# databio/IGD

Measured on AMD Instinct MI355X. Metric: query-intervals/sec (igd search -q, hits-only) on roadmap-scale synthetic .igd, higher is better.
Workload: dtype int32; 1 GPU; BASELINE config 2: roadmap-scale synthetic IGD, 1900 files x 26316 intervals (53143736 tile records, 188505 tiles of 16384 bp, hg38 contigs) replicated per GPU + 1000000 position-sorted queries per step (seed 7), hits-only, queries and DB resident in HBM; queries_per_gpu=1000000, parallelism=query-sharded x1, grouping=sorted, query_layout=contig numbers + starts + ends (12 B/query; igd_hip_search_dev), collective=none

## Files before the change

### igd_amd/csrc/engine/host_search.hpp

```cpp

static int ensure_workspace(igd_hip_db *db, int64_t nq, int pairBytes)
{
    int rc;
    if (nq > db->wsQueries) {
        HIPCHK(hipDeviceSynchronize());
        if (db->d_fix) (void)hipFree(db->d_fix);
        if (db->d_qw) (void)hipFree(db->d_qw);
        if (db->d_later) (void)hipFree(db->d_later);
        if (db->d_laterHdr) (void)hipFree(db->d_laterHdr);
        db->d_fix = nullptr; db->d_qw = nullptr; db->d_later = nullptr; db->d_laterHdr = nullptr;
        db->wsQueries = 0;
        if ((rc = dalloc(&db->d_fix, (size_t)nq * 2, nullptr)) != IGD_HIP_OK) return rc;
        if ((rc = dalloc(&db->d_qw, (size_t)nq + 64, nullptr)) != IGD_HIP_OK) return rc;
        if ((rc = dalloc(&db->d_later, (size_t)nq + 4096 + 64, nullptr)) != IGD_HIP_OK) return rc;
        if ((rc = dalloc(&db->d_laterHdr, 2 * ((size_t)nq / 256 + 2), nullptr)) != IGD_HIP_OK) return rc;
        db->wsQueries = nq;
    }
    if (pairBytes == 0 || (nq <= db->wsBucket && pairBytes <= db->pairBytes)) return IGD_HIP_OK;
    HIPCHK(hipDeviceSynchronize());
    const int64_t cap = nq > db->wsBucket ? nq : db->wsBucket;
    const int pb = pairBytes > db->pairBytes ? pairBytes : db->pairBytes;
    {
        void *ws[] = { db->d_pairs, db->d_long, db->d_spTable, db->d_spT, db->d_spSub };
        for (void *q : ws) if (q) (void)hipFree(q);
// ... 168 lines not shown
                                       int64_t *d_hits, int64_t *d_total, void *stream)
{
    if (!d_run_start || (flags & IGD_HIP_FLAG_BUCKET)) {
        snprintf(g_err, sizeof g_err, "igd_hip_search_runs_dev: bad argument");
        return IGD_HIP_ERR_ARG;
    }
    return search_dev_impl(db, nullptr, d_run_start, d_qs, d_qe, nq, v, rule, flags | IGD_HIP_FLAG_SORTED, d_hits, d_total, stream);
}

static int search_dev_impl(igd_hip_db *db, const int32_t *d_ichr, const int32_t *d_runs, const int32_t *d_qs,
                           const int32_t *d_qe, int64_t nq, int32_t v, int rule, int flags,
                           int64_t *d_hits, int64_t *d_total, void *stream)
{
    if (!db || !d_hits || nq < 0 || nq > IGD_MAX_BATCH || (rule != IGD_HIP_RULE_NEST && rule != IGD_HIP_RULE_FLAT) ||
        ((flags & IGD_HIP_FLAG_SORTED) && (flags & IGD_HIP_FLAG_BUCKET))) {
        snprintf(g_err, sizeof g_err, "igd_hip_search_dev: bad argument");
        return IGD_HIP_ERR_ARG;
    }
    if (db->nFiles == 0) return IGD_HIP_OK;
    if (db->inner) {
        db->inner->vnest = rule == IGD_HIP_RULE_NEST ? 1 : 0;
        return search_dev_impl(db->inner, d_ichr, d_runs, d_qs, d_qe, nq, v, IGD_HIP_RULE_FLAT, flags, d_hits, d_total,
                               stream ? stream : (void *)db->stream);
    }
    HIPCHK(hipSetDevice(db->device));
    hipStream_t st = stream ? (hipStream_t)stream : db->stream;
    if (nq == 0 || db->nT == 0) {
        if (flags & IGD_HIP_FLAG_ZERO_FIRST) {
            HIPCHK(hipMemsetAsync(d_hits, 0, (size_t)db->nFiles * 8, st));
            if (d_total) HIPCHK(hipMemsetAsync(d_total, 0, 8, st));
        }
        return IGD_HIP_OK;
    }
    int rc = ensure_workspace(db, nq, (flags & IGD_HIP_FLAG_SORTED) ? 0 : 8);
    if (rc != IGD_HIP_OK) return rc;
    const bool useV = (v != IGD_HIP_NO_VALUE_FILTER && db->gType == 1);
    const int mode = (flags & IGD_HIP_FLAG_SORTED) ? 1 : (flags & IGD_HIP_FLAG_BUCKET) ? 2 : 0;
    const int krule = rule | ((db->v.vshift >= 0 && db->vnest) ? 0x100 : 0);
    const bool packed = db->packed && !(flags & IGD_HIP_FLAG_EXACT) && (!useV || db->packedV);
    if (db->epoch >= 0x3fffffff || db->covStale) {
        HIPCHK(hipMemsetAsync(db->d_spill, 0, ((size_t)db->nT + 2) * 4, st));
        HIPCHK(hipMemsetAsync(db->d_cov, 0, 4 * IGD_COV_LEN(db->nT) * 4, st));
        HIPCHK(hipMemsetAsync(db->d_ctl + CTL_COV, 0, 4 * 4, st));
        if (db->d_spSub && db->spShift >= 0)
            HIPCHK(hipMemsetAsync(db->d_spSub + (((size_t)db->spCoarse * SPF_S) << db->spShift) + db->spCoarse, 0, (size_t)db->spCoarse * 4, st));
        if (!db->covStale) db->epoch = 0;
        db->covStale = false;
    }
    db->epoch++;
    struct StaleGuard { igd_hip_db *d; bool done; ~StaleGuard() { if (!done) d->covStale = true; } } guard{db, false};
    int slot = -1;
    if (db->evOn && db->evUsed < db->evMax && (db->evSeen++ % (db->evEvery > 0 ? db->evEvery : 1)) == 0) slot = db->evUsed++;
    const bool pipeEv = slot >= 0 && slot < IGD_PIPE_EVENTS;
    if (pipeEv) HIPCHK(hipEventRecord(db->ev[4 * slot + 0], st));
    u64 *zh = (flags & IGD_HIP_FLAG_ZERO_FIRST) ? (u64 *)d_hits : nullptr;
    u64 *zt = (flags & IGD_HIP_FLAG_ZERO_FIRST) ? (u64 *)d_total : nullptr;
    const bool direct = mode == 1 && packed && db->ldsHits && db->nWin == 1 && db->v.tileD != nullptr && db->v.vshift < 0 && db->v.shift >= 0 && db->nCtg <= QB_CTG &&
                        (db->forceDirect > 0 || (db->forceDirect < 0 && (flags & IGD_HIP_FLAG_SHORT) && nq >= 28ll * db->nT));
    db->lastDirect = direct ? 1 : 0;
    if (mode != 2) {
        bool vec = ((((uintptr_t)d_ichr) | ((uintptr_t)d_qs) | ((uintptr_t)d_qe)) & 15) == 0;
        const bool fast = packed && db->v.shift >= 0 && db->nCtg <= QB_CTG;
        if (nq < 65536) vec = false;
        bool runsK = d_runs != nullptr && vec && fast;
        if (d_runs && !runsK) {
            if (nq > db->runCap) {
                HIPCHK(hipStreamSynchronize(st));
                if (db->d_runIchr) (void)hipFree(db->d_runIchr);
                db->d_runIchr = nullptr; db->runCap = 0;
                if ((rc = dalloc(&db->d_runIchr, (size_t)nq, nullptr)) != IGD_HIP_OK) return rc;
                db->runCap = nq;
            }
            k_expand_runs<<<(int)((nq + 255) / 256), 256, 0, st>>>(d_runs, db->nCtg, db->d_runIchr, (int)nq);
            d_ichr = db->d_runIchr;
            vec = vec && (((uintptr_t)d_ichr) & 15) == 0;
        }
        const int fillBlocks = (int)((db->nT >> 10) < 256 ? (db->nT >> 10) + 1 : 256);
        const bool wide = vec && nq >= ((int64_t)1 << 22);
#define QB_GRID(PER_) ((int)((nq + (PER_) - 1) / (PER_)) > fillBlocks ? (int)((nq + (PER_) - 1) / (PER_)) : fillBlocks)
#define QB_LAUNCH(VEC_, FAST_, WGT_)                                                                                                  \
    if (direct && FAST_ && runsK && VEC_ == 4)                                         \
        k_query_bounds<4, true, WGT_, true, true><<<QB_GRID(WGT_ * 4), WGT_, 0, st>>>(db->v, d_runs, d_qs, d_qe, (int)nq, krule,      \
        1, db->d_firstQ, db->d_lpos, db->d_fix, db->d_ctl, db->epoch, zh, zt, db->d_qw, db->d_later, db->d_spill,                      \
        (int2 *)db->d_laterHdr, 1);                                                                                                  \
    else if (direct && FAST_)                                                                                                        \
        k_query_bounds<VEC_, true, WGT_, false, true><<<QB_GRID(WGT_ * VEC_), WGT_, 0, st>>>(db->v, d_ichr, d_qs, d_qe, (int)nq, krule, \
        1, db->d_firstQ, db->d_lpos, db->d_fix, db->d_ctl, db->epoch, zh, zt, db->d_qw, db->d_later, db->d_spill,                      \
        (int2 *)db->d_laterHdr, 1);                                                                                                  \
    else if (runsK && VEC_ == 4 && FAST_)                                                                                             \
        k_query_bounds<4, true, WGT_, true><<<QB_GRID(WGT_ * 4), WGT_, 0, st>>>(db->v, d_runs, d_qs, d_qe, (int)nq, krule,            \
        packed ? 1 : 0, db->d_firstQ, db->d_lpos, db->d_fix, db->d_ctl, db->epoch, zh, zt, db->d_qw, db->d_later, db->d_spill,         \
        (int2 *)db->d_laterHdr, mode == 1 ? 1 : 0);                                                                                  \
    else                                                                                                                             \
    k_query_bounds<VEC_, FAST_, WGT_><<<QB_GRID(WGT_ * VEC_), WGT_, 0, st>>>(db->v, d_ichr, d_qs, d_qe, (int)nq, krule,               \
        packed ? 1 : 0, db->d_firstQ, db->d_lpos, db->d_fix, db->d_ctl, db->epoch, zh, zt, db->d_qw, db->d_later, db->d_spill,         \
        (int2 *)db->d_laterHdr, mode == 1 ? 1 : 0)
        if (wide && !direct) { if (fast) QB_LAUNCH(4, true, 1024); else QB_LAUNCH(4, false, 1024); }
        else if (vec) { if (fast) QB_LAUNCH(4, true, 256); else QB_LAUNCH(4, false, 256); }
        else { if (fast) QB_LAUNCH(1, true, 256); else QB_LAUNCH(1, false, 256); }
#undef QB_LAUNCH
#undef QB_GRID
        db->lbShift = wide ? 12 : vec ? 10 : 8;
    }
    if (mode != 1) {
        if (db->spShift >= 0)
            rc = launch_split(db, d_ichr, d_qs, d_qe, (int)nq, krule, mode == 2 ? 0 : db->epoch, packed ? 1 : 0, st,
                              mode == 2 ? zh : nullptr, mode == 2 ? zt : nullptr);
        else
            rc = launch_bucket(db, d_ichr, d_qs, d_qe, (int)nq, krule, mode == 2 ? 0 : db->epoch, packed ? 1 : 0, st,
                                      mode == 2 ? zh : nullptr, mode == 2 ? zt : nullptr);
        if (rc != IGD_HIP_OK) return rc;
    }
    const bool extEv = slot >= 0 && mode == 1 && packed && db->ldsHits && db->nWin == 1;
    if (slot >= 0 && !extEv) HIPCHK(hipEventRecord(db->ev[4 * slot + 1], st));
    ScanArgs a;
    a.firstQ = db->d_firstQ; a.pairN = db->d_pairN; a.pairPos = db->d_pairPos; a.pairs = (const int2 *)db->d_pairs;
    a.walkList = nullptr; a.ctl = db->d_ctl; a.q_ichr = d_ichr; a.q_qs = d_qs; a.q_qe = d_qe; a.q_w = db->d_qw;
    a.total = (u64 *)d_total; a.hitsOut = (u64 *)d_hits;
    a.nq = (int)nq; a.v = v; a.rule = rule; a.epoch = db->epoch; a.mode = mode;
    a.packedWalk = packed ? (useV ? 2 : 1) : 0;
    const int valves = direct ? 8 : (mode != 1 && packed && db->spShift >= 0 ? 1 : 0) | (mode != 2 && packed ? 2 : 0) |
                       (db->bigImage || db->nRec + IGD_CHUNK >= (1ll << 30) ? 4 : 0);
    const size_t tailWave = direct ? (size_t)IGD_D_WLDS : (size_t)IGD_WLDS_BYTES;
    size_t tailLds = (valves & (2 | 8)) ? (size_t)(db->ldsHits ? IGD_TAIL_WG / IGD_WAVE : 4) * tailWave : 0;
    int tailHistOff = -1;
    if ((size_t)db->nFiles * 8 <= (size_t)48 * 1024) { tailHistOff = (int)tailLds; tailLds += (size_t)db->nFiles * 8; }
    if (db->ldsHits) {
        a.out = db->d_slab;
        const SortK K = make_sortk(db, a);
        for (int win = 0; win < db->nWin; win++) {
            const bool last = win == db->nWin - 1;
            const int fileLo = win * db->winN, fileN = db->nWin == 1 ? db->nFiles : (db->nFiles - fileLo < db->winN ? db->nFiles - fileLo : db->winN);
            if (extEv) { db->evStart = db->ev[4 * slot + 1]; db->evStop = db->ev[4 * slot + 2]; }
            if (direct) {
                DirK D;
                D.db = db->v;
                D.a.firstQ = db->d_firstQ; D.a.tileD = db->v.tileD; D.a.q_qs = d_qs; D.a.q_qe = d_qe; D.a.ctl = db->d_ctl; D.a.fix = db->d_fix;
                D.a.heavyS = db->d_heavy + IGD_HEAVY_MAX; D.a.farList = db->d_far; D.a.nq = (int)nq; D.a.v = v; D.a.epoch = db->epoch;
                D.a.rule = rule; D.a.promised = 1; D.a.sbCap = db->sbCap; D.a.wldsBytes = IGD_D_WLDS + 2 * db->sbCap;
                D.a.out = db->d_slab; D.a.hitsOut = (u64 *)d_hits; D.a.totalOut = (u64 *)d_total;
                if (useV) launch_sorted(db, igd_scan_direct<true>, db->grid, IGD_WG_DIR, (size_t)db->ldsDirect, st, D);
                else launch_sorted(db, igd_scan_direct<false>, db->grid, IGD_WG_DIR, (size_t)db->ldsDirect, st, D);
            } else
            launch_scan_any<true>(db, a, useV, packed, st, db->nWin > 1 ? win : -1);
            if (extEv && db->evStart) {
                db->evStart = db->evStop = nullptr;
                HIPCHK(hipEventRecord(db->ev[4 * slot + 1], st)); HIPCHK(hipEventRecord(db->ev[4 * slot + 2], st));
            }
            if (slot >= 0 && last && !extEv) HIPCHK(hipEventRecord(db->ev[4 * slot + 2], st));
            ScanArgs w = a;
            w.out = (u64 *)d_hits;
            SortK Kt = K;
            Kt.a.sbCap = 0; Kt.a.wldsBytes = (int)tailWave; Kt.a.tailHistOff = tailHistOff;
            const int gx = (fileN + IGD_TAIL_WG - 1) / IGD_TAIL_WG;
            dim3 rg(gx, (!last || IGD_REDUCE_GROUPS * gx >= IGD_TAIL_WGS) ? IGD_REDUCE_GROUPS : (IGD_TAIL_WGS + gx - 1) / gx);
            const int rows32 = (mode != 2 && packed) ? db->epoch : 0;
            if (useV)
                k_reduce_slabs<true><<<rg, IGD_TAIL_WG, last ? tailLds : 0, st>>>(Kt, db->d_slab, db->grid, fileN, (u64 *)d_hits + fileLo, (u64 *)d_total,
                                                               db->d_ctl, mode == 1 ? db->epoch : 0, w, db->d_fix, db->d_long, db->d_heavy, last ? valves : -1, rows32);
            else
                k_reduce_slabs<false><<<rg, IGD_TAIL_WG, last ? tailLds : 0, st>>>(Kt, db->d_slab, db->grid, fileN, (u64 *)d_hits + fileLo, (u64 *)d_total,
                                                                db->d_ctl, mode == 1 ? db->epoch : 0, w, db->d_fix, db->d_long, db->d_heavy, last ? valves : -1, rows32);
        }
    } else {
        a.out = (u64 *)d_hits;
        const SortK K = make_sortk(db, a);
        if (d_total) k_sum_hits<<<1, 256, 0, st>>>((const u64 *)d_hits, db->nFiles, (u64 *)d_total, -1);
        launch_scan_any<false>(db, a, useV, packed, st);
        if (slot >= 0) HIPCHK(hipEventRecord(db->ev[4 * slot + 2], st));
        {
            ScanArgs w = a;
            w.total = nullptr;
            SortK Kt = K;
            Kt.a.sbCap = 0; Kt.a.wldsBytes = IGD_WLDS_BYTES; Kt.a.tailHistOff = tailHistOff;
            if (useV) k_exact_walk<true><<<1024, 256, tailLds, st>>>(Kt, w, db->d_fix, db->d_long, db->d_heavy, valves);
            else k_exact_walk<false><<<1024, 256, tailLds, st>>>(Kt, w, db->d_fix, db->d_long, db->d_heavy, valves);
        }
        if (d_total) k_sum_hits<<<1, 256, 0, st>>>((const u64 *)d_hits, db->nFiles, (u64 *)d_total, +1);
    }
    if (pipeEv) HIPCHK(hipEventRecord(db->ev[4 * slot + 3], st));
    if (mode == 1) db->promised = db->epoch;
    db->lastMode = mode; db->lastPacked = packed ? 1 : 0;
    HIPCHK(hipGetLastError());
    guard.done = true;
    return IGD_HIP_OK;
}

extern "C" int igd_hip_sync(igd_hip_db *db, void *stream)
{
    if (!db) return IGD_HIP_ERR_ARG;
    if (db->inner) return igd_hip_sync(db->inner, stream ? stream : (void *)db->stream);
    HIPCHK(hipSetDevice(db->device));
    HIPCHK(hipStreamSynchronize(stream ? (hipStream_t)stream : db->stream));
    HIPCHK(hipGetLastError());
    if (db->promised) {
        int32_t ctl[4] = {0, 0, 0, 0};
        HIPCHK(hipMemcpy(ctl, db->d_ctl, sizeof ctl, hipMemcpyDeviceToHost));
        const bool broken = ctl[CTL_BROKEN] != 0;
        db->promised = 0;
        if (broken) {
            const int32_t zero = 0;
            HIPCHK(hipMemcpy(db->d_ctl + CTL_BROKEN, &zero, 4, hipMemcpyHostToDevice));
            snprintf(g_err, sizeof g_err, "igd_hip: queries passed with IGD_HIP_FLAG_SORTED were not ordered by "
                     "(contig, start); such a batch added nothing to hits");
            return IGD_HIP_ERR_UNSORTED;
        }
    }
    return IGD_HIP_OK;
}

extern "C" int igd_hip_sync_spin(igd_hip_db *db, void *stream)
{
    if (!db) return IGD_HIP_ERR_ARG;
    HIPCHK(hipSetDevice(db->device));
    hipStream_t st = stream ? (hipStream_t)stream : db->stream;
    for (;;) {
        const hipError_t e = hipStreamQuery(st);
        if (e == hipSuccess) break;
        if (e != hipErrorNotReady) { set_err("hipStreamQuery", e, __FILE__, __LINE__); return IGD_HIP_ERR_DEVICE; }
    }
    return igd_hip_sync(db, stream);
}

static int ensure_qstage(igd_hip_db *db, int64_t nq)
{
    if (nq <= db->qcap) return IGD_HIP_OK;
    HIPCHK(hipDeviceSynchronize());
    if (db->d_qc) (void)hipFree(db->d_qc);
    if (db->d_qs) (void)hipFree(db->d_qs);
    if (db->d_qe) (void)hipFree(db->d_qe);
    db->d_qc = db->d_qs = db->d_qe = nullptr;
    db->qcap = 0;
    int rc;
    if ((rc = dalloc(&db->d_qc, (size_t)nq, nullptr)) != IGD_HIP_OK) return rc;
    if ((rc = dalloc(&db->d_qs, (size_t)nq, nullptr)) != IGD_HIP_OK) return rc;
    if ((rc = dalloc(&db->d_qe, (size_t)nq, nullptr)) != IGD_HIP_OK) return rc;
    db->qcap = nq;
    return IGD_HIP_OK;
}

extern "C" int igd_hip_search(igd_hip_db *db, const int32_t *ichr, const int32_t *qs, const int32_t *qe,
                              int64_t nq, int32_t v, int rule, int64_t *hits, int64_t *total)
{
    return igd_hip_search_ex(db, ichr, qs, qe, nq, v, rule, 0, hits, total);
}

static int search_slab_resident(igd_hip_db *db, const int32_t *ichr, const int32_t *qs, const int32_t *qe,
                                int64_t nq, int32_t v, int rule, int flags)
{
    HIPCHK(hipSetDevice(db->device));
    hipStream_t st = db->stream;
    HIPCHK(hipMemsetAsync(db->d_hits, 0, (size_t)db->nFiles * 8, st));
    HIPCHK(hipMemsetAsync(db->d_total, 0, 8, st));
    const int64_t step = max_batch();
    for (int64_t q0 = 0; q0 < nq; q0 += step) {
        int64_t m = nq - q0 < step ? nq - q0 : step;
        const bool timing = db->timing;
        auto now = []() { struct timespec t; clock_gettime(CLOCK_MONOTONIC, &t); return t.tv_sec * 1e3 + t.tv_nsec * 1e-6; };
        double t0 = now();
        int rc = ensure_qstage(db, m);
        if (rc != IGD_HIP_OK) return rc;
        if (timing) { (void)hipStreamSynchronize(st); fprintf(stderr, "[igd timing]   search: query staging alloc     %7.1f ms\n", now() - t0); t0 = now(); }
        HIPCHK(hipMemcpyAsync(db->d_qc, ichr + q0, (size_t)m * 4, hipMemcpyHostToDevice, st));
        HIPCHK(hipMemcpyAsync(db->d_qs, qs + q0, (size_t)m * 4, hipMemcpyHostToDevice, st));
        HIPCHK(hipMemcpyAsync(db->d_qe, qe + q0, (size_t)m * 4, hipMemcpyHostToDevice, st));
        if (timing) { (void)hipStreamSynchronize(st); fprintf(stderr, "[igd timing]   search: H2D queries             %7.1f ms\n", now() - t0); t0 = now(); }
        rc = igd_hip_search_dev(db, db->d_qc, db->d_qs, db->d_qe, m, v, rule, flags, db->d_hits, db->d_total, st);
        if (rc != IGD_HIP_OK) return rc;
        rc = igd_hip_sync(db, st);
        if (timing) fprintf(stderr, "[igd timing]   search: workspace + kernels        %7.1f ms\n", now() - t0);
        if (rc == IGD_HIP_ERR_UNSORTED) {
            flags &= ~(IGD_HIP_FLAG_SORTED | IGD_HIP_FLAG_SHORT);
            rc = igd_hip_search_dev(db, db->d_qc, db->d_qs, db->d_qe, m, v, rule, flags, db->d_hits, db->d_total, st);
            if (rc == IGD_HIP_OK) rc = igd_hip_sync(db, st);
        }
        if (rc != IGD_HIP_OK) return rc;
    }
    return IGD_HIP_OK;
}

extern "C" int igd_hip_search_ex(igd_hip_db *db, const int32_t *ichr, const int32_t *qs, const int32_t *qe,
                                 int64_t nq, int32_t v, int rule, int flags, int64_t *hits, int64_t *total)
{
    if (!db || !hits || nq < 0 || (nq > 0 && (!ichr || !qs || !qe))) {
        snprintf(g_err, sizeof g_err, "igd_hip_search: bad argument");
        return IGD_HIP_ERR_ARG;
    }
    if (total) *total = 0;
    if (nq == 0 || db->nFiles == 0) return IGD_HIP_OK;
    const int rc = search_slab_resident(db, ichr, qs, qe, nq, v, rule, flags);
    if (rc != IGD_HIP_OK) return rc;
    std::vector<int64_t> h((size_t)db->nFiles);
    int64_t tot = 0;
    HIPCHK(hipMemcpy(h.data(), db->d_hits, (size_t)db->nFiles * 8, hipMemcpyDeviceToHost));
    HIPCHK(hipMemcpy(&tot, db->d_total, 8, hipMemcpyDeviceToHost));
    for (int32_t f = 0; f < db->nFiles; f++) hits[f] += h[f];
    if (total) *total = tot;
    return IGD_HIP_OK;
}
```

### igd_amd/csrc/engine/tail.hpp

```cpp
struct TailHist {
    igd_lds_u64 *p;
    bool on;
    __device__ __forceinline__ void add(int ix, u64 v) const { (void)__hip_atomic_fetch_add(p + ix, v, __ATOMIC_RELAXED, __HIP_MEMORY_SCOPE_WORKGROUP); }
};

template <bool USE_V>
__device__ __forceinline__ void exact_walk_body(const DbView &db, const ScanArgs &a, const int2 *__restrict__ fixList,
                                                const int2 *__restrict__ longList, int gwave, int nwaves, int ctlv, const TailHist hist)
{
    const bool uns = __builtin_amdgcn_readlane(ctlv, CTL_UNSORTED) == a.epoch;
    if (a.mode == 1 && uns) return;
    const bool sortedPath = a.mode == 1 || (a.mode == 0 && !uns);
    const int2 *list = sortedPath ? fixList : longList;
    const int nList = __builtin_amdgcn_readlane(ctlv, (sortedPath ? CTL_NFIX : CTL_NLONG) + (a.epoch & 1));
    const int lane = threadIdx.x & 63;
    u64 found = 0;
    int per = (nList + nwaves - 1) / nwaves;
    per = per > IGD_WAVE ? IGD_WAVE : per;
    for (int l0 = gwave * per; l0 < nList; l0 += nwaves * per) {
        const int cnt = nList - l0 < per ? nList - l0 : per;
        int vq = 0, vkind = -1, vqs = 0, vqe = 0, vn1 = 0, vj1 = -1, vbase = 0, vcnt = 0, voffLo = 0, voffHi = 0, vlob = 0;
        int vu0 = 0, vnu = 0, vqe2 = 0;
        UnitRegs vur;
        vur.offLo = vur.offHi = vur.tile = vur.n = vur.jf = 0;
// ... 236 lines not shown
        const bool cimg = USE_V ? a.packedWalk == 2 : a.packedWalk != 0;
        const int vo2 = lane * 2, vo4 = lane * 4;
        auto issue = [&](int e, Cov &w) {
            w.c = __builtin_amdgcn_readlane(cv, e);
            const int n = __builtin_amdgcn_readlane(ur.n, e);
            const int64_t off = (int64_t)(((unsigned long long)(unsigned)__builtin_amdgcn_readlane(ur.offHi, e) << 32) |
                                          (unsigned)__builtin_amdgcn_readlane(ur.offLo, e));
            if (cimg) {
                const int pre = __builtin_amdgcn_readlane(ur.pre, e);
                const int nrem = n > pre ? n - pre : 0;
                w.nrem = nrem;
                if (USE_V) {
                    const __amdgpu_buffer_rsrc_t rs = __builtin_amdgcn_make_buffer_rsrc((void *)(db.pxv + off + pre), 0, nrem * 4, 0x00020000);
#pragma unroll
                    for (int r = 0; r < IGD_SLOTS; r++) w.ix[r] = (int)__builtin_amdgcn_raw_buffer_load_b32(rs, vo4, r * 256, 0);
                } else {
                    const __amdgpu_buffer_rsrc_t rs = __builtin_amdgcn_make_buffer_rsrc((void *)(db.px + off + pre), 0, nrem * 2, 0x00020000);
#pragma unroll
                    for (int r = 0; r < IGD_SLOTS; r++) w.ix[r] = (int)(unsigned short)__builtin_amdgcn_raw_buffer_load_b16(rs, vo2, r * 128, 0);
                }
                return;
            }
            w.lob = __builtin_amdgcn_readlane(bd, e);
#pragma unroll
            for (int r = 0; r < IGD_SLOTS; r++) {
                const int i = r * IGD_WAVE + lane;
                const int64_t at = off + (i < n ? i : 0);
                const int s0 = db.start[at], x0 = db.idx[at];
                w.st[r] = i < n ? s0 : INT_MIN;
                w.ix[r] = i < n ? x0 : 0;
                if (USE_V) { const int v0 = db.value[at]; w.va[r] = i < n ? v0 : INT_MIN; }
            }
        };
        auto count = [&](const Cov &w) {
            if (cimg) {
                if (!USE_V) found += (u64)(unsigned)w.nrem * (u64)(unsigned)w.c;
#pragma unroll
                for (int r = 0; r < IGD_SLOTS; r++) {
                    if (r * IGD_WAVE >= w.nrem) break;
                    bool in = lane < w.nrem - r * IGD_WAVE;
                    int ix = w.ix[r];
                    if (USE_V) {
                        in = in && (ix >> 16) >= a.v;
                        ix &= 0xFFFF;
                        found += (u64)__popcll(__ballot(in)) * (u64)(unsigned)w.c;
                    }
                    if (in) { if (hist.on) hist.add(ix, (u64)(unsigned)w.c); else atomicAdd(&d_hits[ix], (u64)(unsigned)w.c); }
                }
                return;
            }
#pragma unroll
            for (int r = 0; r < IGD_SLOTS; r++) {
                bool in = w.st[r] >= w.lob;
                if (USE_V) in = in && w.va[r] >= a.v;
                found += (u64)__popcll(__ballot(in)) * (u64)(unsigned)w.c;
                if (in) { if (hist.on) hist.add(w.ix[r], (u64)(unsigned)w.c); else atomicAdd(&d_hits[w.ix[r]], (u64)(unsigned)w.c); }
            }
        };
        Cov C0, C1, C2, C3;
        int e0 = -1, e1 = -1, e2 = -1, e3 = -1;
#define IGD_COV_NEXT(E, C) do { E = -1; if (m) { E = __builtin_ctzll(m); m &= m - 1; issue(E, C); } } while (0)
        IGD_COV_NEXT(e0, C0); IGD_COV_NEXT(e1, C1); IGD_COV_NEXT(e2, C2); IGD_COV_NEXT(e3, C3);
        while (e0 >= 0) {
            count(C0); IGD_COV_NEXT(e0, C0);
            if (e1 >= 0) { count(C1); IGD_COV_NEXT(e1, C1); }
            if (e2 >= 0) { count(C2); IGD_COV_NEXT(e2, C2); }
            if (e3 >= 0) { count(C3); IGD_COV_NEXT(e3, C3); }
            if (e0 < 0) {
                if (e1 >= 0) { count(C1); e1 = -1; }
                if (e2 >= 0) { count(C2); e2 = -1; }
                if (e3 >= 0) { count(C3); e3 = -1; }
            }
        }
#undef IGD_COV_NEXT
    }
    if (d_total && lane == 0 && found) atomicAdd(d_total, found);
}

template <bool USE_V>
__device__ __forceinline__ void batch_tail(const SortK &K, const ScanArgs &wa, const int2 *__restrict__ fixList,
                                           const int2 *__restrict__ longList, const int32_t *__restrict__ heavyB, int valves,
                                           u64 *__restrict__ d_hits, u64 *__restrict__ d_total, unsigned char *smem, int gwave, int nwaves,
                                           int ctlv )
{
    const int lane = threadIdx.x & 63;
    TailHist hist;
    hist.p = (igd_lds_u64 *)(smem + (K.a.tailHistOff >= 0 ? K.a.tailHistOff : 0));
    hist.on = false;
    if (K.a.tailHistOff >= 0) {
        const bool uns = __builtin_amdgcn_readlane(ctlv, CTL_UNSORTED) == wa.epoch;
        const bool sortedPath = wa.mode == 1 || (wa.mode == 0 && !uns);
        const int nList = __builtin_amdgcn_readlane(ctlv, (sortedPath ? CTL_NFIX : CTL_NLONG) + (wa.epoch & 1));
        const bool cov = __builtin_amdgcn_readlane(ctlv, CTL_COV + (sortedPath ? 0 : 2) + (wa.epoch & 1)) == wa.epoch;
        if (!(wa.mode == 1 && uns) && (nList > 0 || cov)) {
            hist.on = true;
            for (int f = threadIdx.x; f < K.db.nFiles; f += blockDim.x) hist.p[f] = 0;
            __syncthreads();
        }
    }
    if (!(IGD_EXP & 0x100000)) exact_walk_body<USE_V>(K.db, wa, fixList, longList, gwave, nwaves, ctlv, hist);
    if (!(IGD_EXP & 0x200000)) coverage_body<USE_V>(K.db, wa, d_hits, d_total, gwave, nwaves, ctlv, hist);
    if (hist.on) {
        __syncthreads();
        for (int f = threadIdx.x; f < K.db.nFiles; f += blockDim.x) {
            const u64 c = hist.p[f];
            if (c) atomicAdd(&d_hits[f], c);
        }
    }
    if (valves & 1) heavy_bucket_body<USE_V>(K.db, wa, heavyB, d_hits, d_total, gwave, nwaves, lane, ctlv);
    if (valves & 8) {
        DirArgs d;
        d.firstQ = K.a.firstQ; d.tileD = K.db.tileD; d.q_qs = wa.q_qs; d.q_qe = wa.q_qe; d.ctl = K.a.ctlw; d.fix = nullptr;
        d.heavyS = K.a.heavyS; d.farList = K.a.farList; d.nq = wa.nq; d.v = wa.v; d.epoch = wa.epoch; d.rule = wa.rule;
        d.promised = 1; d.sbCap = 0; d.wldsBytes = K.a.wldsBytes; d.out = nullptr; d.hitsOut = d_hits; d.totalOut = d_total;
        direct_tail_body<USE_V>(K.db, d, smem + (size_t)(threadIdx.x >> 6) * (size_t)K.a.wldsBytes, gwave, nwaves, lane, ctlv);
    } else
    if (valves & 2) {
        unsigned char *wsm = smem + (size_t)(threadIdx.x >> 6) * (size_t)K.a.wldsBytes;
        if (valves & 4) heavy_sorted_body<USE_V, true>(K, d_hits, d_total, wsm, gwave, nwaves, lane, ctlv);
        else {
            const int par = wa.epoch & 1;
            const bool work = (__builtin_amdgcn_readlane(ctlv, CTL_NHEAVYS + par) | __builtin_amdgcn_readlane(ctlv, CTL_NFAR + par)) != 0 &&
                              __builtin_amdgcn_readlane(ctlv, CTL_UNSORTED) != wa.epoch;
            igd_lds_u64 *lh = (K.a.tailHistOff >= 0 && work) ? hist.p : nullptr;
            if (lh) {
                __syncthreads();
                for (int f = threadIdx.x; f < K.db.nFiles; f += blockDim.x) lh[f] = 0;
                __syncthreads();
            }
            if (!(IGD_EXP & 0x10000)) heavy_sorted_body<USE_V, false>(K, d_hits, d_total, wsm, gwave, nwaves, lane, ctlv, lh);
            if (!(IGD_EXP & 0x20000)) far_units_body<USE_V, false>(K, d_hits, d_total, wsm, gwave, nwaves, lane, ctlv, lh);
            if (lh) {
                __syncthreads();
                for (int f = threadIdx.x; f < K.db.nFiles; f += blockDim.x) {
                    const u64 c = lh[f];
                    if (c) atomicAdd(&d_hits[f], c);
                }
            }
        }
    }
}

template <bool USE_V>
__global__ __launch_bounds__(256) void k_exact_walk(SortK K, ScanArgs a, const int2 *__restrict__ fixList,
                                                    const int2 *__restrict__ longList, const int32_t *__restrict__ heavyB, int valves)
{
    extern __shared__ __attribute__((aligned(16))) unsigned char smem[];
    const int gwave = blockIdx.x * (blockDim.x >> 6) + __builtin_amdgcn_readfirstlane((int)(threadIdx.x >> 6));
    const int ctlv = (threadIdx.x & 63) < IGD_CTL_WORDS ? a.ctl[threadIdx.x & 63] : 0;
    coverage_reset(K.db, a.epoch, gwave, gridDim.x * (blockDim.x >> 6), ctlv);
    batch_tail<USE_V>(K, a, fixList, longList, heavyB, valves, a.out, nullptr, smem, gwave, gridDim.x * (blockDim.x >> 6), ctlv);
}

template <bool USE_V>
__global__ __launch_bounds__(IGD_TAIL_WG) void k_reduce_slabs(SortK K, const u64 *__restrict__ slab, int rows, int nFiles,
                                                      u64 *__restrict__ hits, u64 *__restrict__ total,
                                                      const int32_t *__restrict__ ctl, int brokenIf,
                                                      ScanArgs wa, const int2 *__restrict__ fixList,
                                                      const int2 *__restrict__ longList, const int32_t *__restrict__ heavyB, int valves,
                                                      int rows32 )
{
    extern __shared__ __attribute__((aligned(16))) unsigned char smem[];
    __shared__ u64 red[IGD_TAIL_WG / IGD_WAVE];
    constexpr int WPB = IGD_TAIL_WG / IGD_WAVE;
    const int ctlv = (threadIdx.x & 63) < IGD_CTL_WORDS ? ctl[threadIdx.x & 63] : 0;
    int f = blockIdx.x * IGD_TAIL_WG + threadIdx.x;
    u64 s = 0;
    if (f < nFiles && blockIdx.y < IGD_REDUCE_GROUPS) {
        u64 s64 = 0;
        unsigned long long s32 = 0;
        if (rows32) {
            const unsigned int *slab32 = (const unsigned int *)slab;
            for (int g = blockIdx.y; g < rows; g += IGD_REDUCE_GROUPS) s32 += slab32[(size_t)g * nFiles + f];
            if (__builtin_amdgcn_readlane(ctlv, CTL_UNSORTED) == rows32)
                for (int g = blockIdx.y; g < rows; g += IGD_REDUCE_GROUPS) s64 += slab[(size_t)g * nFiles + f];
            s = __builtin_amdgcn_readlane(ctlv, CTL_UNSORTED) == rows32 ? s64 : s32;
        } else
            for (int g = blockIdx.y; g < rows; g += IGD_REDUCE_GROUPS) s += slab[(size_t)g * nFiles + f];
    }
    if (valves >= 0) coverage_reset(K.db, wa.epoch, (blockIdx.y * gridDim.x + blockIdx.x) * WPB + (int)(threadIdx.x >> 6), gridDim.x * gridDim.y * WPB, ctlv);
    if (brokenIf != 0 && __builtin_amdgcn_readlane(ctlv, CTL_UNSORTED) == brokenIf) return;
    if (s) atomicAdd(&hits[f], s);
    if (total) {
        for (int o = 32; o > 0; o >>= 1) s += __shfl_down(s, o);
        if ((threadIdx.x & 63) == 0) red[threadIdx.x >> 6] = s;
        __syncthreads();
        if (threadIdx.x == 0) {
            u64 t = 0;
            for (int k = 0; k < WPB; k++) t += red[k];
            if (t) atomicAdd(total, t);
        }
    }
    if (valves < 0) return;
    const int nb = gridDim.x * gridDim.y;
    const int bid = blockIdx.y * gridDim.x + blockIdx.x;
    const int gwave = bid * WPB + __builtin_amdgcn_readfirstlane((int)(threadIdx.x >> 6));
    batch_tail<USE_V>(K, wa, fixList, longList, heavyB, valves, wa.out, total, smem, gwave, nb * WPB, ctlv);
}

__global__ __launch_bounds__(256) void k_sum_hits(const u64 *__restrict__ hits, int nFiles,
                                                  u64 *__restrict__ total, int sign)
{
    __shared__ u64 red[4];
    u64 s = 0;
    for (int f = threadIdx.x; f < nFiles; f += 256) s += hits[f];
    for (int o = 32; o > 0; o >>= 1) s += __shfl_down(s, o);
    if ((threadIdx.x & 63) == 0) red[threadIdx.x >> 6] = s;
    __syncthreads();
    if (threadIdx.x == 0) {
        u64 t = red[0] + red[1] + red[2] + red[3];
        if (sign > 0) atomicAdd(total, t);
        else atomicAdd(total, (u64)(-(int64_t)t));
    }
}
```

### igd_amd/csrc/igd_hip.hip

```cpp
#include <hip/hip_runtime.h>
#include <hip/hip_ext.h>
#include <stdint.h>
#include <stdio.h>
#include <stdlib.h>
#include <string.h>
#include <limits.h>
#include <vector>
#include <algorithm>
#include <thread>
#include <mutex>
#include <time.h>
#include <unistd.h>

#include "igd_hip.h"
#include "igd_sortscan.hpp"

#define IGD_WAVE 64
#ifndef IGD_SLOTS
#define IGD_SLOTS 5
#endif
#define IGD_CHUNK (IGD_WAVE * IGD_SLOTS)
#define IGD_SHORT_TILES 4
#ifndef IGD_WPE
#define IGD_WPE 8
#endif
#ifndef IGD_WG
#define IGD_WG 1024
#endif
#define IGD_MAX_BATCH ((long long)IGD_HIP_MAX_BATCH_DEFAULT)
#define IGD_SCAN_ITEMS 16
#define IGD_SCAN_BLOCK 256
#define IGD_SCAN_TILE (IGD_SCAN_ITEMS * IGD_SCAN_BLOCK)
#ifndef IGD_TAIL_WGS
#define IGD_TAIL_WGS 256
#endif
#ifndef IGD_TAIL_WG
#define IGD_TAIL_WG 1024
#endif
#ifndef IGD_REDUCE_GROUPS
#define IGD_REDUCE_GROUPS 64
#endif
#define IGD_PIPE_EVENTS 16
#define IGD_WINDOW_FILES 10240
#define IGD_MAX_WINDOWS 16
#define IGD_LDS_HITS_MAX_BYTES (120 * 1024)

typedef unsigned long long u64;

#ifndef IGD_EXP_NOMATCH
#define IGD_EXP_NOMATCH 0
#endif

#ifndef IGD_EXP
#define IGD_EXP 0
#endif

static thread_local char g_err[512] = "";
static void set_err(const char *what, hipError_t e, const char *file, int line)
{
    snprintf(g_err, sizeof g_err, "%s: %s (%s:%d)", what, hipGetErrorString(e), file, line);
}
#define HIPCHK(call)                                                          \
    do {                                                                      \
        hipError_t e_ = (call);                                               \
        if (e_ != hipSuccess) {                                               \
            set_err(#call, e_, __FILE__, __LINE__);                           \
            return IGD_HIP_ERR_DEVICE;                                        \
        }                                                                     \
    } while (0)

extern "C" const char *igd_hip_last_error(void) { return g_err; }
extern "C" void igd_hip_set_error_(const char *msg) { snprintf(g_err, sizeof g_err, "%s", msg); }

extern "C" int igd_hip_device_count(void)
{
    int n = 0;
    hipError_t e = hipGetDeviceCount(&n);
    if (e != hipSuccess) {
        set_err("hipGetDeviceCount", e, __FILE__, __LINE__);
        return 0;
    }
    return n;
}

static int64_t max_batch(void)
{
    static const int64_t m = []() -> int64_t {
        return igd_hip_max_batch_rule(getenv("IGD_HIP_MAX_BATCH"));
    }();
    return m;
}
extern "C" int64_t igd_hip_max_batch(void) { return max_batch(); }

#define IGD_EXP_WRONG_BITS (1 | 2 | 4 | 8 | 64 | 128 | 256 | 512 | 8192 | 0x10000 | 0x20000 | 0x40000 | 0x80000 | 0x100000 | 0x200000 | 0x800000)
extern "C" unsigned igd_hip_build_flags(void) { return ((unsigned)IGD_EXP & 0xffffffu) | (IGD_EXP_NOMATCH ? 1u << 24 : 0u); }
extern "C" unsigned igd_hip_build_wrong_counts(void);

struct __attribute__((aligned(16))) Unit {
    int64_t off;
    int32_t tile;
    int32_t n;
    int32_t jf;
    uint32_t W[6];
    int32_t pre;
};
#define UNIT_J(u) ((u).jf >> 4)
#define UNIT_FLAGS(u) ((u).jf & 15)

struct SpTuple { int32_t t, s, e; };

struct DbView {
    int32_t nbp, shift, nCtg, nT, nUnits, nFiles;
    const Unit *units;
    const int32_t *start, *end, *idx, *value;
    const uint32_t *pse;
    const uint16_t *px;
    const uint32_t *pxv;
    const int64_t *tileOff;
    const int32_t *tileCnt;
    const int32_t *tileBd;
    const int32_t *ctgBase;
    const int32_t *ctgNTile;
    const int32_t *tileUnit0;
    int32_t *cov;
    const uint32_t *tileBits;
    const int4 *tileD;
    int32_t vshift;
    const int32_t *rNTile, *rBase;
    const uint32_t *rEmpty;
    int32_t fileLo;
};

struct igd_hip_db {
    int device;
    int32_t nbp, gType, nCtg, nFiles, nT;
    int64_t nRec;
    DbView v;
    int32_t *d_start, *d_end, *d_idx, *d_value;
    uint32_t *d_pse;
    uint16_t *d_px;
    uint32_t *d_pxv;
    bool packed, packedV;
    int64_t *d_tileOff;
    int32_t *d_tileCnt, *d_tileBd, *d_ctgBase, *d_ctgNTile, *d_tileUnit0;
    int32_t *d_heavy;
    int32_t *d_far;
    Unit *d_units;
    int32_t nUnits;
    int64_t resident;
    int32_t *d_firstQ, *d_pairN;
    int32_t *d_lpos;
    int32_t *d_cov;
    bool covStale;
    igd_hip_db *inner;
    uint32_t *d_rEmpty;
    int vnest;
    int32_t *d_runIchr;
    int64_t runCap;
    int32_t *d_qw;
    int32_t *d_later;
    int32_t *d_spill;
    int ldsSorted;
    int32_t maxTileCnt;
    int sbCap;
    int32_t *d_laterHdr;
    int lbShift;
    int lastMode, lastPacked;
    int forceRank;
    int forceDirect;
    int4 *d_tileD;
    uint32_t *d_tileBits;
    int ldsDirect;
    int lastDirect;
    bool bigImage;
    bool timing;
    bool splitNoStage, splitNoBits, splitNoRegion;
    uint32_t *d_spTable;
    SpTuple *d_spT;
    uint32_t *d_spSub;
    int spShift, spCoarse;
    char *arena;
    size_t arenaSize, arenaUsed;
    int32_t epoch;
    int32_t promised;
    int32_t *d_pairCnt, *d_pairPos, *d_blockSums;
    void *d_pairs;
    int2 *d_long, *d_fix;
    int32_t *d_ctl;
    int64_t wsQueries;
    int64_t wsBucket;
    int pairBytes;
    u64 *d_slab;
    int grid, ldsBytes;
    bool ldsHits;
// ... 93 lines not shown
```

Baseline: 12.56 billion query-intervals/s.

## Restructure slab reduction: wave-per-file-column split with unrolled loads and LDS combine

Reworks k_reduce_slabs so each workgroup owns a 64-file column strip, split across IGD_REDUCE_SPLIT workgroups and the waves within each one. Row loads are unrolled IGD_REDUCE_DEPTH deep to keep more memory requests in flight, and partial sums are combined in LDS before a single atomic per file, which cuts global atomic traffic. The grid becomes 1D, sized from the file count, with a minimum when the batch tail runs. The tail work now runs before the final combine, and tail/summing work is divided by block id differently, which may change load balance.

```diff
diff --git a/igd_amd/csrc/engine/host_search.hpp b/igd_amd/csrc/engine/host_search.hpp
--- a/igd_amd/csrc/engine/host_search.hpp
+++ b/igd_amd/csrc/engine/host_search.hpp
@@ -344,8 +344,8 @@
             w.out = (u64 *)d_hits;
             SortK Kt = K;
             Kt.a.sbCap = 0; Kt.a.wldsBytes = (int)tailWave; Kt.a.tailHistOff = tailHistOff;
-            const int gx = (fileN + IGD_TAIL_WG - 1) / IGD_TAIL_WG;
-            dim3 rg(gx, (!last || IGD_REDUCE_GROUPS * gx >= IGD_TAIL_WGS) ? IGD_REDUCE_GROUPS : (IGD_TAIL_WGS + gx - 1) / gx);
+            const int sumWgs = (fileN + IGD_WAVE - 1) / IGD_WAVE * IGD_REDUCE_SPLIT;
+            dim3 rg(last && sumWgs < IGD_TAIL_WGS ? IGD_TAIL_WGS : sumWgs);
             const int rows32 = (mode != 2 && packed) ? db->epoch : 0;
             if (useV)
                 k_reduce_slabs<true><<<rg, IGD_TAIL_WG, last ? tailLds : 0, st>>>(Kt, db->d_slab, db->grid, fileN, (u64 *)d_hits + fileLo, (u64 *)d_total,
diff --git a/igd_amd/csrc/engine/tail.hpp b/igd_amd/csrc/engine/tail.hpp
--- a/igd_amd/csrc/engine/tail.hpp
+++ b/igd_amd/csrc/engine/tail.hpp
@@ -412,6 +412,23 @@
     batch_tail<USE_V>(K, a, fixList, longList, heavyB, valves, a.out, nullptr, smem, gwave, gridDim.x * (blockDim.x >> 6), ctlv);
 }
 
+template <typename T>
+__device__ __forceinline__ u64 column_share(const T *__restrict__ slab, int rows, int nFiles, int file, int first, int step)
+{
+    u64 s = 0;
+    for (int g0 = first; g0 < rows; g0 += IGD_REDUCE_DEPTH * step) {
+        T v[IGD_REDUCE_DEPTH];
+#pragma unroll
+        for (int k = 0; k < IGD_REDUCE_DEPTH; k++) {
+            const int g = g0 + k * step;
+            v[k] = slab[(size_t)(g < rows ? g : g0) * nFiles + file];
+        }
+#pragma unroll
+        for (int k = 0; k < IGD_REDUCE_DEPTH; k++) s += g0 + k * step < rows ? (u64)v[k] : 0;
+    }
+    return s;
+}
+
 template <bool USE_V>
 __global__ __launch_bounds__(IGD_TAIL_WG) void k_reduce_slabs(SortK K, const u64 *__restrict__ slab, int rows, int nFiles,
                                                       u64 *__restrict__ hits, u64 *__restrict__ total,
@@ -421,41 +438,44 @@
                                                       int rows32 )
 {
     extern __shared__ __attribute__((aligned(16))) unsigned char smem[];
-    __shared__ u64 red[IGD_TAIL_WG / IGD_WAVE];
     constexpr int WPB = IGD_TAIL_WG / IGD_WAVE;
+    __shared__ u64 part[WPB * IGD_WAVE];
     const int ctlv = (threadIdx.x & 63) < IGD_CTL_WORDS ? ctl[threadIdx.x & 63] : 0;
-    int f = blockIdx.x * IGD_TAIL_WG + threadIdx.x;
-    u64 s = 0;
-    if (f < nFiles && blockIdx.y < IGD_REDUCE_GROUPS) {
-        u64 s64 = 0;
-        unsigned long long s32 = 0;
-        if (rows32) {
-            const unsigned int *slab32 = (const unsigned int *)slab;
-            for (int g = blockIdx.y; g < rows; g += IGD_REDUCE_GROUPS) s32 += slab32[(size_t)g * nFiles + f];
-            if (__builtin_amdgcn_readlane(ctlv, CTL_UNSORTED) == rows32)
-                for (int g = blockIdx.y; g < rows; g += IGD_REDUCE_GROUPS) s64 += slab[(size_t)g * nFiles + f];
-            s = __builtin_amdgcn_readlane(ctlv, CTL_UNSORTED) == rows32 ? s64 : s32;
-        } else
-            for (int g = blockIdx.y; g < rows; g += IGD_REDUCE_GROUPS) s += slab[(size_t)g * nFiles + f];
-    }
-    if (valves >= 0) coverage_reset(K.db, wa.epoch, (blockIdx.y * gridDim.x + blockIdx.x) * WPB + (int)(threadIdx.x >> 6), gridDim.x * gridDim.y * WPB, ctlv);
-    if (brokenIf != 0 && __builtin_amdgcn_readlane(ctlv, CTL_UNSORTED) == brokenIf) return;
-    if (s) atomicAdd(&hits[f], s);
-    if (total) {
-        for (int o = 32; o > 0; o >>= 1) s += __shfl_down(s, o);
-        if ((threadIdx.x & 63) == 0) red[threadIdx.x >> 6] = s;
-        __syncthreads();
-        if (threadIdx.x == 0) {
-            u64 t = 0;
-            for (int k = 0; k < WPB; k++) t += red[k];
-            if (t) atomicAdd(total, t);
-        }
-    }
-    if (valves < 0) return;
     const int nb = gridDim.x * gridDim.y;
     const int bid = blockIdx.y * gridDim.x + blockIdx.x;
-    const int gwave = bid * WPB + __builtin_amdgcn_readfirstlane((int)(threadIdx.x >> 6));
-    batch_tail<USE_V>(K, wa, fixList, longList, heavyB, valves, wa.out, total, smem, gwave, nb * WPB, ctlv);
+    const int wave = __builtin_amdgcn_readfirstlane((int)(threadIdx.x >> 6)), lane = threadIdx.x & 63;
+    const bool summing = bid < (nFiles + IGD_WAVE - 1) / IGD_WAVE * IGD_REDUCE_SPLIT;
+    const int f = bid / IGD_REDUCE_SPLIT * IGD_WAVE + lane;
+    if (summing) {
+        const int fc = f < nFiles ? f : nFiles - 1;
+        const int first = bid % IGD_REDUCE_SPLIT + IGD_REDUCE_SPLIT * wave, step = IGD_REDUCE_SPLIT * WPB;
+        u64 s;
+        if (rows32) {
+            s = column_share((const unsigned int *)slab, rows, nFiles, fc, first, step);
+            if (__builtin_amdgcn_readlane(ctlv, CTL_UNSORTED) == rows32)
+                s = column_share(slab, rows, nFiles, fc, first, step);
+        } else
+            s = column_share(slab, rows, nFiles, fc, first, step);
+        part[wave * IGD_WAVE + lane] = f < nFiles ? s : 0;
+    }
+    if (valves >= 0) coverage_reset(K.db, wa.epoch, bid * WPB + wave, nb * WPB, ctlv);
+    const bool broken = brokenIf != 0 && __builtin_amdgcn_readlane(ctlv, CTL_UNSORTED) == brokenIf;
+    if (broken) return;
+    if (valves >= 0)
+        batch_tail<USE_V>(K, wa, fixList, longList, heavyB, valves, wa.out, total, smem, bid * WPB + wave, nb * WPB, ctlv);
+    if (summing) {
+        __syncthreads();
+        if (wave == 0) {
+            u64 t = 0;
+#pragma unroll
+            for (int k = 0; k < WPB; k++) t += part[k * IGD_WAVE + lane];
+            if (t) atomicAdd(&hits[f], t);
+            if (total) {
+                for (int o = 32; o > 0; o >>= 1) t += __shfl_down(t, o);
+                if (lane == 0 && t) atomicAdd(total, t);
+            }
+        }
+    }
 }
 
 __global__ __launch_bounds__(256) void k_sum_hits(const u64 *__restrict__ hits, int nFiles,
diff --git a/igd_amd/csrc/igd_hip.hip b/igd_amd/csrc/igd_hip.hip
--- a/igd_amd/csrc/igd_hip.hip
+++ b/igd_amd/csrc/igd_hip.hip
@@ -37,9 +37,12 @@
 #ifndef IGD_TAIL_WG
 #define IGD_TAIL_WG 1024
 #endif
-#ifndef IGD_REDUCE_GROUPS
-#define IGD_REDUCE_GROUPS 64
-#endif
+#ifndef IGD_REDUCE_SPLIT
+#define IGD_REDUCE_SPLIT 4
+#endif
+static_assert(IGD_REDUCE_SPLIT >= 1 && IGD_REDUCE_SPLIT <= 32 && (IGD_REDUCE_SPLIT & (IGD_REDUCE_SPLIT - 1)) == 0, "IGD_REDUCE_SPLIT: a power of two, 1 .. 32");
+#define IGD_REDUCE_DEPTH (512 / (IGD_REDUCE_SPLIT * (IGD_TAIL_WG / IGD_WAVE)))
+static_assert(IGD_REDUCE_DEPTH >= 1, "IGD_REDUCE_DEPTH: column_share's loop would not advance");
 #define IGD_PIPE_EVENTS 16
 #define IGD_WINDOW_FILES 10240
 #define IGD_MAX_WINDOWS 16
```

Measured after the change: 12.90 billion query-intervals/s, median of 6. 2.7% higher.
